# amacati/gp-mpc

Hardware: AMD Instinct MI355X
Metric: GP-MPC control steps/sec, 2D quadrotor H=30 N=200, batch 1024 @1/2/4/8 GPU (higher is better)
Workload: dtype f64

## Files before the change

gp-mpc_amd/csrc/capi.hip:

```cpp
#include "../../include/gpmpc_mi355x.h"

#include <cmath>
#include <cstdio>
#include <cstdlib>
#include <cstring>
#include <string>
#include <unordered_map>
#include <vector>

#include "gp_tile.h"
#include "gpmpc_common.h"

using namespace gpmpc;

static_assert(GPMPC_STATS_SLOTS == kStatsSlots, "public stats-slot count must match the kernel's");

#ifndef GPMPC_VAR_TRIM_DEFAULT
#define GPMPC_VAR_TRIM_DEFAULT 1
#endif

namespace {
thread_local std::string g_err;

gpmpc_status fail(gpmpc_status s, const std::string& msg) {
    g_err = msg;
    return s;
}

#define HIPCHK(expr)                                                                        \
    do {                                                                                    \
        hipError_t e_ = (expr);                                                             \
        if (e_ != hipSuccess)                                                               \
            return fail(GPMPC_ERR_HIP, std::string(#expr) + ": " + hipGetErrorString(e_));   \
    } while (0)

struct ModelDims {
    int nx, nu, ngp, nparams;
    int gp_dim[kMaxGP];
    int var_src[kMaxGP][3];
};

bool model_dims(int id, ModelDims& m) {
    switch (id) {
        case kQuad2D:
            m = ModelDims{6, 2, 2, 6, {1, 3, 0, 0}, {{6, 0, 0}, {4, 5, 7}, {0, 0, 0}, {0, 0, 0}}};
            return true;
        case kQuad3D:
            m = ModelDims{12, 4, 3, 9, {1, 3, 3, 0}, {{0, 0, 0}, {1, 2, 3}, {4, 5, 6}, {0, 0, 0}}};
            return true;
        case kCartpole:
            m = ModelDims{4, 1, 2, 4, {3, 3, 0, 0}, {{2, 3, 4}, {2, 3, 4}, {0, 0, 0}, {0, 0, 0}}};
            return true;
// ... 117 lines not shown
    int32_t* has_prev = nullptr;
    double* lin = nullptr;
    int32_t* lin_tag = nullptr;
    int32_t* t_prev = nullptr;
    bool lin_cache = true;
    int32_t* order = nullptr;
    uint32_t* cost = nullptr;
    double* traj = nullptr;
    double* tgain = nullptr;
    GPSlot gp[kMaxGP];
    bool profiling = false;
    std::vector<hipEvent_t> ev_pool;
    std::unordered_map<hipEvent_t, bool> ev_fenced;
    std::vector<std::pair<hipEvent_t, hipEvent_t>> ev_var, ev_sqp;
    std::vector<hipEvent_t> ev_var_owned;
    unsigned long long* timing = nullptr;
    long long* stats = nullptr;
    int32_t* scratch_i = nullptr;
    double* scratch_d = nullptr;
    double* obs = nullptr;
    double* roll = nullptr;
    size_t roll_doubles = 0;
    double* sel = nullptr;
    size_t sel_rows[kMaxGP] = {0, 0, 0, 0};
    double* red = nullptr;
    size_t red_rows = 0, red_m = 0;
    int var_batch = 0;
    hipStream_t last_stream = nullptr;
    hipEvent_t ev_last = nullptr;
    bool ev_last_valid = false;
    bool tail_unmarked = false;
    bool overlap = true;
    int var_split = 0;
    bool var_trim = GPMPC_VAR_TRIM_DEFAULT != 0;
    bool event_fence = false;
    double* stage_cost = nullptr;
    hipStream_t side = nullptr;
    hipEvent_t ev_fork = nullptr, ev_join = nullptr;
    int tail = -1;
};

static hipError_t order_after_last(gpmpc_handle* h, hipStream_t s) {
    if (!h->ev_last) {
        const hipError_t e = hipEventCreateWithFlags(&h->ev_last, hipEventDisableTiming);
        if (e != hipSuccess) {
            h->ev_last = nullptr;
            return e;
        }
    }
    if (h->last_stream == s) return hipSuccess;
    if (h->tail_unmarked) {
        if (hipEventRecord(h->ev_last, h->last_stream) == hipSuccess) {
            h->ev_last_valid = true;
        } else {
            (void)hipGetLastError();
            (void)hipStreamSynchronize(h->last_stream);
            (void)hipGetLastError();
        }
        h->tail_unmarked = false;
    }
    if (h->ev_last_valid) return hipStreamWaitEvent(s, h->ev_last, 0);
    return hipSuccess;
}
struct StreamMark {
    gpmpc_handle* h;
    hipStream_t s;
    ~StreamMark() {
// ... 1145 lines not shown
    HIPCHK(hipMemcpyAsync(h->u, u_dev, B * H * h->md.nu * sizeof(double), hipMemcpyDeviceToDevice, s));
    bump_lin(h);
    HIPCHK(hipMemsetAsync(h->t_prev, 0xff, B * sizeof(int32_t), s));
    HIPCHK(hipMemsetAsync(h->pi, 0, B * H * h->md.nx * sizeof(double), s));
    HIPCHK(hipMemsetAsync(h->lam, 0, B * (H + 1) * 2 * h->nb * sizeof(double), s));
    return GPMPC_OK;
}

gpmpc_status gpmpc_solve(gpmpc_handle* h, int32_t batch, const double* x0, const int32_t* tstep, double* u0,
                         int32_t* status, int32_t* sqp_iter, int32_t* qp_iter, double* res, void* stream) {
    if (!h) return fail(GPMPC_ERR_ARG, "null handle");
    if (!h->model_set) return fail(GPMPC_ERR_STATE, "gpmpc_set_model not called");
    if (!h->ref_set) return fail(GPMPC_ERR_STATE, "gpmpc_set_reference not called");
    if (batch < 1 || batch > h->max_batch) return fail(GPMPC_ERR_ARG, "batch out of range");
    if (!x0 || !tstep || !u0 || !status) return fail(GPMPC_ERR_ARG, "null output/input");
    if (h->P.tighten && h->P.use_gp)
        for (int g = 0; g < h->md.ngp; ++g)
            if (!h->gp[g].linvT) return fail(GPMPC_ERR_STATE, "tightening needs Linv for every GP");
    (void)hipSetDevice(h->device);
    hipStream_t s = (hipStream_t)stream;
    HIPCHK(order_after_last(h, s));
    StreamMark mark{h, s};
    ProblemDev P = h->P;
    P.tighten = (h->P.tighten && h->P.use_gp) ? 1 : 0;
    auto give_back = [&](hipEvent_t& e) {
        if (e) h->ev_pool.push_back(e);
        e = nullptr;
    };
    auto launch_var = [&](int first, int count, const int32_t* order, hipStream_t st) -> hipError_t {
        PostBatch pb{};
        pb.n = h->md.ngp;
        pb.step_points = batch * h->H;
        pb.var_split = h->var_split;
        pb.var_full = h->var_trim ? 0 : 1;
        for (int g = 0; g < h->md.ngp; ++g) {
            PostArgs& a = pb.a[g];
            a.sx = h->x;
            a.su = h->u;
            a.H = h->H;
            a.nx = h->md.nx;
            a.nu = h->md.nu;
            a.ngp = h->md.ngp;
            a.gp_index = g;
            for (int k = 0; k < 3; ++k) a.src[k] = h->md.var_src[g][k];
            a.P = count * h->H;
            a.d = h->md.gp_dim[g];
            a.with_noise = 1;
            a.mean = nullptr;
            a.var = h->var;
            a.var_stride = h->md.ngp;
            a.var_off = g;
            a.order = order;
            a.first = first;
            pb.g[g] = P.gp[g];
            pb.g[g].vroot = h->gp[g].vroot;
            pb.g[g].vroot_cols = h->gp[g].vroot_cols;
            pb.g[g].vroot_rank = h->gp[g].vroot_rank;
            pb.npad[g] = h->gp[g].npad;
        }
        return launch_gp_post_batch(pb, true, st);
    };
    StateDev S{h->x, h->u, h->pi, h->lam, h->has_prev, h->var, h->tight, h->lin_cache ? h->lin : nullptr, h->lin_tag,
               h->order, h->cost, 0, h->t_prev};
    StepIO io{x0, tstep, u0, status, sqp_iter, qp_iter, res, h->timing, h->stats};
    if (!io.sqp_iter) io.sqp_iter = h->scratch_i;
    if (!io.qp_iter) io.qp_iter = h->scratch_i + h->max_batch;
    if (!io.res) io.res = h->scratch_d;
// ... 155 lines not shown
    }
    return GPMPC_OK;
}

gpmpc_status gpmpc_get_launch_segments(gpmpc_handle* h, int32_t batch, int32_t* segments) {
    if (!h) return fail(GPMPC_ERR_ARG, "null handle");
    if (batch < 1 || batch > h->max_batch) return fail(GPMPC_ERR_ARG, "batch out of range");
    if (!segments) return fail(GPMPC_ERR_ARG, "null output");
    *segments = sqp_launch_segments(h->P, batch);
    return GPMPC_OK;
}

gpmpc_status gpmpc_set_tuning(gpmpc_handle* h, int32_t option, int32_t value) {
    if (!h) return fail(GPMPC_ERR_ARG, "null handle");
    switch (option) {
        case GPMPC_TUNE_LIN_CACHE:
            if (value != 0 && value != 1) break;
            if (h->lin_cache != (value == 1)) bump_lin(h);
            h->lin_cache = value == 1;
            return GPMPC_OK;
        case GPMPC_TUNE_ORDER:
            if (value < 0 || value > 2) break;
            h->P.order_dispatch = value;
            return GPMPC_OK;
        case GPMPC_TUNE_OVERLAP:
            if (value != 0 && value != 1) break;
            h->overlap = value == 1;
            return GPMPC_OK;
        case GPMPC_TUNE_VAR_SPLIT:
            if (value != 0 && value != 1 && value != 4) break;
            h->var_split = value;
            return GPMPC_OK;
        case GPMPC_TUNE_VAR_TRIM:
            if (value != 0 && value != 1) break;
            h->var_trim = value == 1;
            return GPMPC_OK;
        case GPMPC_TUNE_SEG:
            if (value != 0 && value != 1) break;
            h->P.seg = value;
            return GPMPC_OK;
        case GPMPC_TUNE_SEG_PIVOT:
            if (value < -1 || value > 300) break;
            h->P.seg_piv_rel = value < 0 ? HUGE_VAL : std::pow(10.0, -value);
            return GPMPC_OK;
        case GPMPC_TUNE_TAIL:
            if (value < -1 || value > 16384) break;
            h->tail = value;
            return GPMPC_OK;
        case GPMPC_TUNE_SHIFT:
            if (value != 0 && value != 1) break;
            h->P.shift = value;
            return GPMPC_OK;
        case GPMPC_TUNE_EVENT_FENCE:
            if (value != 0 && value != 1) break;
            if (h->event_fence != (value == 1)) {
                for (hipEvent_t e : h->ev_pool) {
                    h->ev_fenced.erase(e);
                    (void)hipEventDestroy(e);
                }
                h->ev_pool.clear();
            }
            h->event_fence = value == 1;
            return GPMPC_OK;
        default:
            return fail(GPMPC_ERR_ARG, "unknown tuning option " + std::to_string(option));
    }
    return fail(GPMPC_ERR_ARG, "bad value " + std::to_string(value) + " for tuning option " + std::to_string(option));
}
// ... 104 lines not shown

gpmpc_status gpmpc_gp_predict(gpmpc_handle* h, int32_t gp_id, const double* Z, int32_t P, double* mean, double* var,
                              int32_t with_noise, void* stream) {
    if (!h) return fail(GPMPC_ERR_ARG, "null handle");
    if (gp_id < 0 || gp_id >= h->md.ngp || !h->gp[gp_id].set) return fail(GPMPC_ERR_STATE, "GP not set");
    if (P < 0 || (P > 0 && !Z)) return fail(GPMPC_ERR_ARG, "bad points");
    if (var && !h->gp[gp_id].linvT) return fail(GPMPC_ERR_STATE, "variance needs Linv");
    if (P == 0) return GPMPC_OK;
    (void)hipSetDevice(h->device);
    hipStream_t s = (hipStream_t)stream;
    HIPCHK(order_after_last(h, s));
    StreamMark mark{h, s};
    const GPDev& g = h->P.gp[gp_id];
    PostArgs a{};
    a.Z = Z;
    a.ldz = h->md.gp_dim[gp_id];
    a.P = P;
    a.d = h->md.gp_dim[gp_id];
    a.with_noise = with_noise;
    a.var_stride = 1;
    a.var_off = 0;
    if (mean) {
        GPDev gm = g;
        gm.vrows = g.rows;
        gm.nv = g.n;
        gm.linvT = nullptr;
        a.mean = mean;
        a.var = nullptr;
        HIPCHK(launch_gp_post(gm, (g.n + 15) / 16 * 16, a, false, s));
    }
    if (var) {
        a.mean = nullptr;
        a.var = var;
        HIPCHK(launch_gp_post(g, h->gp[gp_id].npad, a, false, s, h->var_trim ? 0 : 1));
    }
    return GPMPC_OK;
}

gpmpc_status gpmpc_gp_mean_grad(gpmpc_handle* h, int32_t gp_id, const double* Z, int32_t P, double* mean,
                                double* grad, void* stream) {
    if (!h) return fail(GPMPC_ERR_ARG, "null handle");
    if (gp_id < 0 || gp_id >= h->md.ngp || !h->gp[gp_id].set) return fail(GPMPC_ERR_STATE, "GP not set");
    if (P < 0 || (P > 0 && !Z)) return fail(GPMPC_ERR_ARG, "bad points");
    if (P == 0) return GPMPC_OK;
    (void)hipSetDevice(h->device);
    hipStream_t s = (hipStream_t)stream;
    HIPCHK(order_after_last(h, s));
    StreamMark mark{h, s};
    HIPCHK(launch_gp_mean_grad(h->P.gp[gp_id], Z, P, mean, grad, s));
    return GPMPC_OK;
}

gpmpc_status gpmpc_gp_posterior(int32_t n, int32_t d, int32_t npad, const double* rows, const double* linvT,
                                double lengthscale, double outputscale, double noise, const double* Z, int32_t P,
                                double* mean, double* var, int32_t with_noise, void* stream) {
    if (n < 1 || d < 1 || d > kMaxGPDim || npad < n || npad % 16 != 0 || !rows)
        return fail(GPMPC_ERR_ARG, "bad GP layout (need 1 <= d <= 3, npad = 16-multiple >= n)");
    if (P < 0 || (P > 0 && !Z)) return fail(GPMPC_ERR_ARG, "bad points");
    if (var && !linvT) return fail(GPMPC_ERR_ARG, "variance needs linvT");
    if (!(lengthscale > 0.0) || !(outputscale > 0.0) || !(noise >= 0.0)) return fail(GPMPC_ERR_ARG, "bad hyperparameters");
    if (P == 0) return GPMPC_OK;
    GPDev g{};
    g.rows = rows;
    g.vrows = rows;
    g.linvT = linvT;
    g.n = g.nv = n;
    g.d = d;
// ... 65 lines not shown
    const hipError_t e = hipMalloc(&fresh, doubles * sizeof(double));
    if (e != hipSuccess) return fail(GPMPC_ERR_NOMEM, std::string("hipMalloc: ") + hipGetErrorString(e));
    if (*buf) (void)hipFree(*buf);
    *buf = fresh;
    return GPMPC_OK;
}

static gpmpc_status ensure_observe_scratch(gpmpc_handle* h) {
    return h->obs ? GPMPC_OK : replace_scratch(&h->obs, observe_layout(h).end);
}

struct PointVariances {
    const double* Z;
    int32_t ldz;
    const double* var;
    int32_t ldv;
};
static gpmpc_status queue_point_variances(gpmpc_handle* h, int32_t P, const double* x_dev, const double* u_dev,
                                          hipStream_t s, PointVariances* out) {
    const ObserveLayout lay = observe_layout(h);
    GPObserve a = observe_args(h, P, x_dev, u_dev, nullptr, P, nullptr, 1.0, 0.0);
    a.inputs = h->obs + lay.zin;
    HIPCHK(launch_gp_observe(a, s));
    for (int g = 0, col = 0; g < h->md.ngp; col += h->md.gp_dim[g], ++g) {
        PostArgs pa{};
        pa.Z = h->obs + lay.zin + col;
        pa.ldz = (int)lay.D;
        pa.P = P;
        pa.d = h->md.gp_dim[g];
        pa.with_noise = 0;
        pa.var = h->obs + lay.var + (size_t)g * h->max_batch;
        pa.var_stride = 1;
        pa.var_off = 0;
        HIPCHK(launch_gp_post(h->P.gp[g], h->gp[g].npad, pa, false, s, h->var_trim ? 0 : 1));
    }
    *out = PointVariances{h->obs + lay.zin, (int32_t)lay.D, h->obs + lay.var, h->max_batch};
    return GPMPC_OK;
}

gpmpc_status gpmpc_preprocess(gpmpc_handle* h, int32_t P, const double* x_dev, const double* u_dev,
                              const double* xnext_dev, int32_t m, const int32_t* pick_dev, double dt_diff,
                              double gravity, double* inputs_dev, double* targets_dev, void* stream) {
    if (!h) return fail(GPMPC_ERR_ARG, "null handle");
    const char* bad = transitions_bad(P, x_dev, u_dev, xnext_dev, m, pick_dev, dt_diff, gravity);
    if (!bad && !inputs_dev && !targets_dev) bad = "no output (inputs_dev and targets_dev both NULL)";
    if (bad) return fail(GPMPC_ERR_ARG, bad);
    if (!h->model_set) return fail(GPMPC_ERR_STATE, "the prior parameters are not set (gpmpc_set_model first)");
    (void)hipSetDevice(h->device);
    GPObserve a = observe_args(h, P, x_dev, u_dev, xnext_dev, m, pick_dev, dt_diff, gravity);
    a.inputs = inputs_dev;
    a.targets = targets_dev;
    HIPCHK(launch_gp_observe(a, (hipStream_t)stream));
    return GPMPC_OK;
}

gpmpc_status gpmpc_gp_informative(gpmpc_handle* h, int32_t P, const double* x_dev, const double* u_dev, int32_t m,
                                  int32_t* pick_dev, double* score_dev, void* stream) {
    if (!h) return fail(GPMPC_ERR_ARG, "null handle");
    if (P < 1 || P > h->max_batch) return fail(GPMPC_ERR_ARG, "P must be in 1 .. max_batch");
    if (m < 1 || m > P) return fail(GPMPC_ERR_ARG, "m must be in 1 .. P");
    if (!x_dev || !u_dev || !pick_dev) return fail(GPMPC_ERR_ARG, "null points or picks");
    for (int g = 0; g < h->md.ngp; ++g) {
        if (!h->gp[g].set) return fail(GPMPC_ERR_STATE, "GP not set (gpmpc_set_gp first)");
        if (!h->gp[g].linvT) return fail(GPMPC_ERR_STATE, "the variance needs Linv (the GP was set without it)");
    }
    (void)hipSetDevice(h->device);
    const gpmpc_status got = ensure_observe_scratch(h);
// ... 242 lines not shown
    const size_t need = var_dev ? (size_t)P * T * D : 0;
    if (need > h->roll_doubles) {
        const gpmpc_status got = replace_scratch(&h->roll, need);
        if (got != GPMPC_OK) return got;
        h->roll_doubles = need;
    }
    HIPCHK(ensure_side(h));
    hipStream_t s = h->side;
    HIPCHK(order_after_last(h, s));
    StreamMark mark{h, s};
    RolloutArgs a{};
    for (int i = 0; i < kMaxParams; ++i) a.params[i] = h->P.params[i];
    a.dt = h->P.dt;
    a.P = P;
    a.T = T;
    a.x0 = x0_dev;
    a.u = u_dev;
    a.x = x_dev;
    if (with_gp)
        for (int g = 0; g < ngp; ++g) a.gp[g] = h->P.gp[g];
    HIPCHK(launch_rollout(h->model, a, with_gp != 0, s));
    if (var_dev) {
        HIPCHK(launch_rollout_inputs(h->model, x_dev, u_dev, P, T, h->roll, s));
        for (int g = 0, col = 0; g < ngp; col += h->md.gp_dim[g], ++g) {
            PostArgs pa{};
            pa.Z = h->roll + col;
            pa.ldz = (int)D;
            pa.P = P * T;
            pa.d = h->md.gp_dim[g];
            pa.with_noise = 0;
            pa.var = var_dev;
            pa.var_stride = ngp;
            pa.var_off = g;
            HIPCHK(launch_gp_post(h->P.gp[g], h->gp[g].npad, pa, false, s, h->var_trim ? 0 : 1));
        }
    }
    HIPCHK(hipStreamSynchronize(s));
    return GPMPC_OK;
}

gpmpc_status gpmpc_rollout_lin(gpmpc_handle* h, int32_t P, int32_t T, const double* x0_dev, const double* u_dev,
                               int32_t with_gp, double* x_dev, double* A_dev, double* B_dev, double* var_dev,
                               const double* K, const double* cov0_dev, int32_t with_noise, double* cov_dev) {
    if (!h) return fail(GPMPC_ERR_ARG, "null handle");
    const int nx = h->md.nx, nu = h->md.nu;
    const char* bad = nullptr;
    if (P < 1 || T < 1) bad = "no trajectories or no steps (P, T >= 1)";
    else if (!x0_dev || !u_dev || !x_dev) bad = "null array (x0_dev, u_dev and x_dev are required)";
    else if (!A_dev || !B_dev) bad = "null array (A_dev and B_dev are required)";
    else if (with_gp != 0 && with_gp != 1) bad = "with_gp must be 0 or 1";
    else if (with_noise != 0 && with_noise != 1) bad = "with_noise must be 0 or 1";
    else if ((int64_t)P * ((int64_t)T + 1) * nx > INT32_MAX) bad = "P (T + 1) nx does not fit an int32";
    else if ((int64_t)P * (int64_t)T * nx * nx > INT32_MAX) bad = "P T nx nx does not fit an int32";
    if (!bad && K)
        for (int i = 0; i < nu * nx; ++i)
            if (!std::isfinite(K[i])) bad = "K has a non-finite entry";
    if (bad) return fail(GPMPC_ERR_ARG, bad);
    if (!h->model_set) return fail(GPMPC_ERR_STATE, "the prior parameters are not set (gpmpc_set_model first)");
    const int ngp = h->md.ngp;
    if (with_gp) {
        if (!h->P.use_gp) return fail(GPMPC_ERR_STATE, "with_gp = 1 while the handle's GPs are off (gpmpc_use_gp)");
        for (int g = 0; g < ngp; ++g)
            if (!h->gp[g].set) return fail(GPMPC_ERR_STATE, "GP " + std::to_string(g) + " not set");
    }
    const bool want_var = var_dev || cov_dev;
    if (want_var)
        for (int g = 0; g < ngp; ++g) {
// ... 10 lines not shown
        if (got != GPMPC_OK) return got;
        h->roll_doubles = need;
    }
    HIPCHK(ensure_side(h));
    hipStream_t s = h->side;
    HIPCHK(order_after_last(h, s));
    StreamMark mark{h, s};
    RolloutLinArgs a{};
    for (int i = 0; i < kMaxParams; ++i) a.r.params[i] = h->P.params[i];
    a.r.dt = h->P.dt;
    a.r.P = P;
    a.r.T = T;
    a.r.x0 = x0_dev;
    a.r.u = u_dev;
    a.r.x = x_dev;
    a.A = A_dev;
    a.B = B_dev;
    if (with_gp)
        for (int g = 0; g < ngp; ++g) a.r.gp[g] = h->P.gp[g];
    HIPCHK(launch_rollout_lin(h->model, a, with_gp != 0, s));
    if (want_var) {
        double* var = var_dev ? var_dev : h->roll + gathered;
        HIPCHK(launch_rollout_inputs(h->model, x_dev, u_dev, P, T, h->roll, s));
        for (int g = 0, col = 0; g < ngp; col += h->md.gp_dim[g], ++g) {
            PostArgs pa{};
            pa.Z = h->roll + col;
            pa.ldz = (int)D;
            pa.P = P * T;
            pa.d = h->md.gp_dim[g];
            pa.with_noise = 0;
            pa.var = var;
            pa.var_stride = ngp;
            pa.var_off = g;
            HIPCHK(launch_gp_post(h->P.gp[g], h->gp[g].npad, pa, false, s, h->var_trim ? 0 : 1));
        }
        if (cov_dev) {
            RolloutCovArgs c{};
            c.dt = h->P.dt;
            c.P = P;
            c.T = T;
            c.closed = K ? 1 : 0;
            if (K)
                for (int i = 0; i < nu * nx; ++i) c.K[i] = K[i];
            for (int g = 0; g < ngp; ++g) c.noise[g] = with_noise ? h->P.gp[g].sn2 : 0.0;
            c.x = x_dev;
            c.u = u_dev;
            c.A = A_dev;
            c.B = B_dev;
            c.var = var;
            c.cov0 = cov0_dev;
            c.cov = cov_dev;
            HIPCHK(launch_rollout_cov(h->model, c, s));
        }
    }
    HIPCHK(hipStreamSynchronize(s));
    return GPMPC_OK;
}

gpmpc_status gpmpc_rollout_sample(gpmpc_handle* h, int32_t P, int32_t T, const double* x0_dev, const double* u_dev,
                                  const double* xref_dev, const double* K, int32_t clip, const double* xi_dev,
                                  int32_t with_gp, int32_t with_noise, double* x_dev, double* uapp_dev,
                                  double* var_dev) {
    if (!h) return fail(GPMPC_ERR_ARG, "null handle");
    const int nx = h->md.nx, nu = h->md.nu;
    const char* bad = nullptr;
    if (P < 1 || T < 1) bad = "no trajectories or no steps (P, T >= 1)";
    else if (!x0_dev || !u_dev || !x_dev) bad = "null array (x0_dev, u_dev and x_dev are required)";
// ... 62 lines not shown
```

gp-mpc_amd/csrc/gp_kernels.hip:

```cpp
#include "gpmpc_common.h"
#include "models.h"

#include <algorithm>
#include <atomic>
#include <type_traits>

namespace gpmpc {

typedef double f64x4 __attribute__((ext_vector_type(4)));


template <bool FROM_STATE>
__device__ __forceinline__ void load_point(const PostArgs& a, int p, double (&z)[3]) {
    if (FROM_STATE) {
        const int r = p / a.H, k = p - r * a.H;
        const int b = a.order ? a.order[a.first + r] : r;
#pragma unroll
        for (int dd = 0; dd < 3; ++dd) {
            const int s = a.src[dd];
            z[dd] = (dd < a.d) ? (s < a.nx ? a.sx[((size_t)b * (a.H + 1) + k) * a.nx + s]
                                           : a.su[((size_t)b * a.H + k) * a.nu + (s - a.nx)])
                               : 0.0;
        }
    } else {
#pragma unroll
        for (int dd = 0; dd < 3; ++dd) z[dd] = (dd < a.d) ? a.Z[(size_t)p * a.ldz + dd] : 0.0;
    }
}

constexpr int kPostWaves = 8;
constexpr int kMaxCT = 16;

__device__ __forceinline__ double dpp_quad_sum(double v) {
    auto mv = [](double x, auto ctrl) {
        const long long b = __double_as_longlong(x);
        const int lo = __builtin_amdgcn_update_dpp(0, (int)b, decltype(ctrl)::value, 0xf, 0xf, false);
        const int hi = __builtin_amdgcn_update_dpp(0, (int)(b >> 32), decltype(ctrl)::value, 0xf, 0xf, false);
        return __longlong_as_double(((long long)hi << 32) | (unsigned int)lo);
    };
    v += mv(v, std::integral_constant<int, 0x4E>{});
    v += mv(v, std::integral_constant<int, 0xB1>{});
    return v;
}

__host__ __device__ inline int post_ct(int npad) { return npad / 16 < kMaxCT ? npad / 16 : kMaxCT; }
__host__ __device__ inline int post_stride(int ct) { return 16 * (ct | 1); }

template <bool FROM_STATE, bool FULL>
__global__ __launch_bounds__(64 * kPostWaves) void gp_post_kernel(PostBatch pb) {
    extern __shared__ __attribute__((aligned(16))) double panel[];
    const GPDev& g = pb.g[blockIdx.y];
    const PostArgs& a = pb.a[blockIdx.y];
    const int npad = pb.npad[blockIdx.y];
    if ((int)blockIdx.x * kPostWaves * 16 >= a.P) return;
    const int tid = threadIdx.x;
    const int lane = tid & 63, wave = tid >> 6;
    const int lc = lane & 15;
    const int kq = lane >> 4;
    const int p0 = (blockIdx.x * kPostWaves + wave) * 16;
    const int p = p0 + lc;
    const bool pvalid = p < a.P;
    double z[3];
    load_point<FROM_STATE>(a, pvalid ? p : a.P - 1, z);
    const double c = -0.5 * g.inv_ell2;
    const double4* rows = reinterpret_cast<const double4*>(g.vrows);
    double msum = 0.0;
    auto kval = [&](int i, bool acc_mean) {
        double kv = 0.0;
        if (i < g.nv) {
            const double4 r = rows[i];
            const double xr[3] = {r.x, r.y, r.z};
            double q = 0.0;
#pragma unroll
            for (int dd = 0; dd < 3; ++dd) {
                const double df = (dd < g.d) ? xr[dd] - z[dd] : 0.0;
                q = fma(df, df, q);
// ... 453 lines not shown
    const PostArgs a = pb.a[blockIdx.y];
    const int npad = pb.npad[blockIdx.y];
    const int lane = threadIdx.x & 63, wave = threadIdx.x >> 6;
    const int p0 = (blockIdx.x * kLoveWaves + wave) * 16;
    if (p0 >= a.P) return;
    int nf, nq;
    love_tiles(g.vroot_rank, nf, nq);
    love_dispatch<1, FROM_STATE>(3 * nf + nq, g, a, npad, p0, lane);
}

template <bool FROM_STATE>
hipError_t launch_love(const PostBatch& pb, hipStream_t stream) {
    int blocks = 0;
    for (int q = 0; q < pb.n; ++q) blocks = max(blocks, (pb.a[q].P + 16 * kLoveWaves - 1) / (16 * kLoveWaves));
    hipLaunchKernelGGL((gp_love_kernel<FROM_STATE>), dim3(blocks, pb.n), dim3(64 * kLoveWaves), 0, stream, pb);
    return hipGetLastError();
}

template <int NT, bool FROM_STATE, int NQ>
hipError_t launch_var_tri_nq(const PostBatch& pb, int blocks, hipStream_t stream) {
    static bool attr = false;
    const int lds = 2 * 16 * 16 * (NT | 1) * (int)sizeof(double);
    if (!attr) {
        const hipError_t e = hipFuncSetAttribute((const void*)gp_var_tri_kernel<NT, FROM_STATE, NQ>,
                                                 hipFuncAttributeMaxDynamicSharedMemorySize, lds);
        if (e != hipSuccess) return e;
        attr = true;
    }
    hipLaunchKernelGGL((gp_var_tri_kernel<NT, FROM_STATE, NQ>), dim3(blocks, pb.n), dim3(64 * kPostWaves), lds, stream, pb);
    return hipGetLastError();
}

static int var_tri_quads(const PostBatch& pb, int ntile) {
    if (pb.var_full) return 0;
    int nr = 0;
    for (int q = 0; q < pb.n; ++q) {
        const int r = pb.g[q].nv - 16 * (ntile - 1);
        if (r < 1 || r > 8) return 0;
        nr = std::max(nr, r);
    }
    return (nr + 3) / 4;
}

template <bool FROM_STATE, int NT = 1>
hipError_t launch_var_tri(const PostBatch& pb, int ntile, int blocks, int split, hipStream_t stream) {
    if constexpr (NT <= kMaxCT) {
        if (ntile == NT) {
            if (split == 4) {
                static bool sattr = false;
                const int lds = var_split_lds(NT, split);
                auto* k = gp_var_split_kernel<NT, FROM_STATE, 4>;
                if (!sattr) {
                    const hipError_t e = hipFuncSetAttribute((const void*)k, hipFuncAttributeMaxDynamicSharedMemorySize, lds);
                    if (e != hipSuccess) return e;
                    sattr = true;
                }
                const int pts = 16 * (kPostWaves / split);
                int sblocks = 0;
                for (int q = 0; q < pb.n; ++q) sblocks = std::max(sblocks, (pb.a[q].P + pts - 1) / pts);
                hipLaunchKernelGGL(k, dim3(sblocks, pb.n), dim3(64 * kPostWaves), lds, stream, pb);
                return hipGetLastError();
            }
            switch (var_tri_quads(pb, NT)) {
                case 1: return launch_var_tri_nq<NT, FROM_STATE, 1>(pb, blocks, stream);
                case 2: return launch_var_tri_nq<NT, FROM_STATE, 2>(pb, blocks, stream);
                default: return launch_var_tri_nq<NT, FROM_STATE, 0>(pb, blocks, stream);
            }
        }
        return launch_var_tri<FROM_STATE, NT + 1>(pb, ntile, blocks, split, stream);
    }
    return hipErrorInvalidValue;
}

hipError_t launch_gp_post_batch(const PostBatch& pb, bool from_state, hipStream_t stream) {
    int blocks = 0;
    size_t lds = 0;
    for (int q = 0; q < pb.n; ++q) {
        blocks = max(blocks, (pb.a[q].P + 16 * kPostWaves - 1) / (16 * kPostWaves));
        if (pb.a[q].var != nullptr && (pb.g[q].linvT != nullptr || pb.g[q].vroot != nullptr)) {
            const int ncols = pb.g[q].vroot ? pb.g[q].vroot_cols : pb.npad[q];
            lds = std::max(lds, (size_t)2 * 16 * post_stride(post_ct(ncols)) * sizeof(double));
        }
    }
    if (blocks == 0 || pb.n == 0) return hipSuccess;
    bool love = true;
    for (int q = 0; q < pb.n; ++q) {
        love = love && pb.a[q].mean == nullptr && pb.a[q].var != nullptr && pb.g[q].vroot != nullptr &&
               pb.g[q].vroot_cols % 16 == 0 && pb.g[q].vroot_cols <= 16 * kLoveMaxTiles &&
               pb.g[q].vroot_rank >= 1 && pb.g[q].vroot_rank <= pb.g[q].vroot_cols;
    }
    if (love)
        return from_state ? launch_love<true>(pb, stream) : launch_love<false>(pb, stream);
    bool tri = true;
    for (int q = 0; q < pb.n; ++q)
        tri = tri && pb.a[q].mean == nullptr && pb.a[q].var != nullptr && pb.g[q].linvT != nullptr &&
// ... 5 lines not shown
                n = 256;
            return n;
        }();
        const int step_blocks = pb.step_points > 0 ? (pb.step_points + 16 * kPostWaves - 1) / (16 * kPostWaves) : blocks;
        const int wgs = step_blocks * pb.n;
        int split = 2 * wgs <= ncu ? 4 : 1;
        if (pb.var_split == 1 || pb.var_split == 4) split = pb.var_split;
        return from_state ? launch_var_tri<true>(pb, pb.npad[0] / 16, blocks, split, stream)
                          : launch_var_tri<false>(pb, pb.npad[0] / 16, blocks, split, stream);
    }
    static std::atomic<bool> attr{false};
    if (!attr.load(std::memory_order_acquire)) {
        const int mx = 2 * 16 * post_stride(kMaxCT) * (int)sizeof(double);
        for (const void* k : {(const void*)gp_post_kernel<true, false>, (const void*)gp_post_kernel<false, false>,
                              (const void*)gp_post_kernel<true, true>, (const void*)gp_post_kernel<false, true>}) {
            const hipError_t e = hipFuncSetAttribute(k, hipFuncAttributeMaxDynamicSharedMemorySize, mx);
            if (e != hipSuccess) return e;
        }
        attr.store(true, std::memory_order_release);
    }
    bool full = true;
    for (int q = 0; q < pb.n; ++q) {
        const bool var = pb.a[q].var != nullptr && (pb.g[q].linvT != nullptr || pb.g[q].vroot != nullptr);
        const int ncols = pb.g[q].vroot ? pb.g[q].vroot_cols : pb.npad[q];
        full = full && (!var || post_ct(ncols) == kMaxCT);
    }
    auto* k = from_state ? (full ? gp_post_kernel<true, true> : gp_post_kernel<true, false>)
                         : (full ? gp_post_kernel<false, true> : gp_post_kernel<false, false>);
    hipLaunchKernelGGL(k, dim3(blocks, pb.n), dim3(64 * kPostWaves), lds, stream, pb);
    return hipGetLastError();
}

hipError_t launch_gp_post(const GPDev& g, int npad, const PostArgs& a, bool from_state, hipStream_t stream,
                          int var_full) {
    PostBatch pb{};
    pb.var_full = var_full;
    pb.g[0] = g;
    pb.a[0] = a;
    pb.npad[0] = npad;
    pb.n = 1;
    return launch_gp_post_batch(pb, from_state, stream);
}

template <int ID>
__global__ void plant_step_kernel(PlantParams params, double dt, const double* __restrict__ x,
                                  const double* __restrict__ u, double* __restrict__ xn, int32_t* tstep, int B) {
    using M = Model<ID>;
    constexpr int NX = M::NX, NU = M::NU;
    const int b = blockIdx.x * blockDim.x + threadIdx.x;
    if (b >= B) return;
    double p[kMaxParams];
#pragma unroll
    for (int i = 0; i < kMaxParams; ++i) p[i] = params.v[i];
    double xs[NX], us[NU], k[NX], acc[NX], xi[NX];
    const double gm[kMaxGP] = {0.0, 0.0, 0.0, 0.0};
#pragma unroll
    for (int i = 0; i < NX; ++i) xs[i] = x[(size_t)b * NX + i];
#pragma unroll
    for (int a = 0; a < NU; ++a) us[a] = u[(size_t)b * NU + a];
    const double cs[4] = {0.0, 0.5, 0.5, 1.0}, ws[4] = {1.0, 2.0, 2.0, 1.0};
#pragma unroll
    for (int s = 0; s < 4; ++s) {
#pragma unroll
        for (int i = 0; i < NX; ++i) xi[i] = (s == 0) ? xs[i] : fma(cs[s] * dt, k[i], xs[i]);
        M::f(p, xi, us, gm, k);
#pragma unroll
        for (int i = 0; i < NX; ++i) acc[i] = (s == 0) ? k[i] : fma(ws[s], k[i], acc[i]);
    }
#pragma unroll
// ... 18 lines not shown
```

gp-mpc_amd/csrc/gpmpc_common.h:

```cpp
#pragma once
#include <hip/hip_runtime.h>
#include <cstdint>
#include <type_traits>

namespace gpmpc {

constexpr int kMaxGP = 4;
constexpr int kMaxGPDim = 3;
constexpr int kMaxNX = 12;
constexpr int kMaxNU = 4;
constexpr int kMaxH = 63;
constexpr int kPhases = 15;
constexpr int kMaxParams = 16;
constexpr int kStatsSlots = 12;
constexpr double kSlackMin = 1e-12;

enum ModelId : int32_t { kQuad2D = 0, kQuad3D = 1, kCartpole = 2 };

enum SolveStatus : int32_t { kSuccess = 0, kNaN = 1, kMaxIter = 2, kMinStep = 3, kQPFailure = 4 };

struct GPDev {
    const double* rows;
    const double* vrows;
    const double* linvT;
// ... 116 lines not shown
    p = fma(p, r, 0.5000000000000019);
    p = fma(p, r, 1.0);
    p = fma(p, r, 1.0);
    return __hiloint2double(__double2hiint(p) + (__double2loint(t) << 20), __double2loint(p));
}

template <int K>
__device__ __forceinline__ void exp_rbf_n(double (&x)[K]) {
    constexpr double kMagic = 6755399441055744.0;
    constexpr double c[12] = {2.5110037605963777e-08, 2.763263963904103e-07, 2.755724091857897e-06,
                              2.4801485482328494e-05, 0.00019841269890047113, 0.0013888888952314775,
                              0.008333333333319601, 0.0416666666664881, 0.1666666666666668,
                              0.5000000000000019, 1.0, 1.0};
    double t[K], r[K], p[K];
#pragma unroll
    for (int k = 0; k < K; ++k) x[k] = exp_rbf_clamp(x[k]);
#pragma unroll
    for (int k = 0; k < K; ++k) t[k] = fma(x[k], 1.4426950408889634, kMagic);
#pragma unroll
    for (int k = 0; k < K; ++k) r[k] = fma(t[k] - kMagic, -6.93147180369123816490e-01, x[k]);
#pragma unroll
    for (int k = 0; k < K; ++k) r[k] = fma(t[k] - kMagic, -1.90821492927058770002e-10, r[k]);
#pragma unroll
    for (int k = 0; k < K; ++k) p[k] = fma(c[0], r[k], c[1]);
#pragma unroll
    for (int i = 2; i < 12; ++i)
#pragma unroll
        for (int k = 0; k < K; ++k) p[k] = fma(p[k], r[k], c[i]);
#pragma unroll
    for (int k = 0; k < K; ++k)
        x[k] = __hiloint2double(__double2hiint(p[k]) + (__double2loint(t[k]) << 20), __double2loint(p[k]));
}

__device__ __forceinline__ double dpp_row_sum(double v) {
    auto mv = [](double x, auto ctrl) {
        const long long b = __double_as_longlong(x);
        const int lo = __builtin_amdgcn_update_dpp(0, (int)b, decltype(ctrl)::value, 0xf, 0xf, false);
        const int hi = __builtin_amdgcn_update_dpp(0, (int)(b >> 32), decltype(ctrl)::value, 0xf, 0xf, false);
        return __longlong_as_double(((long long)hi << 32) | (unsigned int)lo);
    };
    v += mv(v, std::integral_constant<int, 0x128>{});
    v += mv(v, std::integral_constant<int, 0x124>{});
    v += mv(v, std::integral_constant<int, 0x4E>{});
    v += mv(v, std::integral_constant<int, 0xB1>{});
    return v;
}

struct PostBatch {
    GPDev g[kMaxGP];
    PostArgs a[kMaxGP];
    int32_t npad[kMaxGP];
    int32_t n;
    int32_t step_points;
    int32_t var_split;
    int32_t var_full;
};

struct GPAppend {
    double* rows;
    double* tX;
    double* tW;
    double* linvT;
    int32_t npad;
    int32_t n0;
    int32_t m;
    int32_t d;
    double xbar[3];
    double inv_ell2, sf2, sn2;
    const double* Xnew;
    const double* ynew;
    double* wt;
    int32_t ldw;
    double* pmean;
    double* lbinv;
    double* beta;
    int32_t* flag;
    int32_t* accepted;
};

struct GPDrop {
    const double* src;
    double* dst;
    const double* rows;
    const double* tX;
    double* srows;
    double* stX;
    double* stW;
    int32_t npad0;
// ... 262 lines not shown
    const double* linvT;
    int32_t nv, npad;
    double inv_ell2, sf2;
};
struct RolloutSampleArgs {
    RolloutArgs r;
    const double* xref;
    const double* xi;
    double* uapp;
    double* var;
    int32_t closed, clip;
    double K[kMaxNU * kMaxNX];
    double u_lo[kMaxNU], u_hi[kMaxNU];
    double noise[kMaxGP];
    RolloutSampleGP vg[kMaxGP];
};
hipError_t launch_rollout_sample(int model, const RolloutSampleArgs& a, bool with_gp, hipStream_t stream);
struct RolloutCovArgs {
    double dt;
    int32_t P, T;
    int32_t closed;
    double K[kMaxNU * kMaxNX];
    double noise[kMaxGP];
    const double* x;
    const double* u;
    const double* A;
    const double* B;
    const double* var;
    const double* cov0;
    double* cov;
};
hipError_t launch_rollout_cov(int model, const RolloutCovArgs& a, hipStream_t stream);
hipError_t launch_gp_post(const GPDev& g, int npad, const PostArgs& a, bool from_state, hipStream_t stream,
                          int var_full = 0);
hipError_t launch_gp_post_batch(const PostBatch& pb, bool from_state, hipStream_t stream);
struct PlantParams {
    double v[kMaxParams];
};
hipError_t launch_plant(int model, const PlantParams& params, double dt, const double* x, const double* u, double* xn,
                        int32_t* tstep, int B, hipStream_t stream);

}
```

gp-mpc_amd/gpmpc/_lib.py:

```python

from __future__ import annotations

import ctypes
import hashlib
import os
from ctypes import POINTER, c_char_p, c_double, c_int32, c_int64, c_void_p
from pathlib import Path

import torch

_DEFAULT_LIB = Path(__file__).resolve().parent / "lib" / "libgpmpc_mi355x.so"
LIB_PATH = Path(os.environ.get("GPMPC_LIB", _DEFAULT_LIB))
CSRC = Path(__file__).resolve().parents[1] / "csrc"
HASHED = ["sqp_kernel.hip", "gp_kernels.hip", "gp_append.hip", "gp_drop.hip", "gp_refactor.hip", "gp_fit.hip",
          "gp_love.hip", "gp_fitc.hip", "gp_observe.hip", "rollout_cov.hip", "capi.hip", "gpmpc_common.h", "gp_tile.h", "gp_pick.h",
          "models.h", "../../include/gpmpc_mi355x.h", "build_id.cpp", "Makefile"]

_lib = None

_D = c_double
_I = c_int32
_P = c_void_p
SIGNATURES = {
    "gpmpc_create": (_I, [_I, _I, _I, _I, POINTER(_P)]),
    "gpmpc_destroy": (None, [_P]),
    "gpmpc_last_error": (c_char_p, []),
    "gpmpc_set_model": (_I, [_P, _P, _I, _D, _P, _P, _P, _P, _P, _P, _P, _D, _I]),
    "gpmpc_set_reference": (_I, [_P, _P, _I]),
    "gpmpc_set_options": (_I, [_P, _I, _D, _D, _D, _D, _I, _D, _D]),
    "gpmpc_set_gp": (_I, [_P, _I, _I, _I, _P, _P, _I, _P, _P, _D, _D, _D]),
    "gpmpc_gp_reserve": (_I, [_P, _I, _I]),
    "gpmpc_gp_append": (_I, [_P, _I, _I, _P, _P, _P, _P]),
    "gpmpc_gp_drop_oldest": (_I, [_P, _I, _I, _P, _P]),
    "gpmpc_gp_drop_rows": (_I, [_P, _I, _I, _P, _P, _P, _P]),
    "gpmpc_gp_refactor": (_I, [_P, _I, _P, _D, _D, _D, _P, _P]),
    "gpmpc_gp_mll": (_I, [_P, _I, _P, _P, _P]),
    "gpmpc_gp_fit": (_I, [_P, _I, _P, _D, _I, POINTER(_D), POINTER(_I), POINTER(_I), _P, _P]),
    "gpmpc_gp_love_root": (_I, [_P, _I, _I, _P, POINTER(_I), POINTER(_I), _P]),
    "gpmpc_get_gp_variance_root": (_I, [_P, _I, POINTER(_I), POINTER(_I), _P, _P]),
    "gpmpc_gp_fitc": (_I, [_P, _I, _I, _P, _P, _D, POINTER(_I), _P]),
    "gpmpc_get_gp_fitc": (_I, [_P, _I, POINTER(_I), _P, _P, _P]),
    "gpmpc_gp_inducing": (_I, [_P, _I, _I, _D, _P, _P, _P, POINTER(_I)]),
    "gpmpc_gp_size": (_I, [_P, _I, POINTER(_I), POINTER(_I)]),
    "gpmpc_use_gp": (_I, [_P, _I]),
    "gpmpc_set_gp_variance_root": (_I, [_P, _I, _I, _I, _P]),
    "gpmpc_set_tightening": (_I, [_P, _I, _D, _P, _P, _P]),
    "gpmpc_set_var_inputs": (_I, [_P, _I, _P, _I]),
    "gpmpc_reset": (_I, [_P, _I, _I, _P]),
# ... 96 lines not shown
```

Before: 3.193 million.

## Add quad-tiled MFMA variance kernel and make it the default trim mode

Adds a new GP posterior-variance kernel that computes the triangular solve product with 4x4x4 f64 MFMA over quad-sized column blocks. It double-buffers Linv panels in LDS and interleaves the RBF kernel-vector evaluation for the next tile with the current tile's MFMAs. A third var_trim mode (2) selects it and becomes the new default. This is meant to cut the wasted work and latency of the older triangular/full variance paths, at the cost of more register pressure, more template instantiations, and a new code path that must match the old numerics.

```diff
diff --git a/gp-mpc_amd/csrc/capi.hip b/gp-mpc_amd/csrc/capi.hip
--- a/gp-mpc_amd/csrc/capi.hip
+++ b/gp-mpc_amd/csrc/capi.hip
@@ -14,10 +14,6 @@
 using namespace gpmpc;
 
 static_assert(GPMPC_STATS_SLOTS == kStatsSlots, "public stats-slot count must match the kernel's");
-
-#ifndef GPMPC_VAR_TRIM_DEFAULT
-#define GPMPC_VAR_TRIM_DEFAULT 1
-#endif
 
 namespace {
 thread_local std::string g_err;
@@ -201,7 +197,7 @@
     bool tail_unmarked = false;
     bool overlap = true;
     int var_split = 0;
-    bool var_trim = GPMPC_VAR_TRIM_DEFAULT != 0;
+    int var_trim = GPMPC_VAR_TRIM_DEFAULT;
     bool event_fence = false;
     double* stage_cost = nullptr;
     hipStream_t side = nullptr;
@@ -1413,7 +1409,7 @@
         pb.n = h->md.ngp;
         pb.step_points = batch * h->H;
         pb.var_split = h->var_split;
-        pb.var_full = h->var_trim ? 0 : 1;
+        pb.var_trim = h->var_trim;
         for (int g = 0; g < h->md.ngp; ++g) {
             PostArgs& a = pb.a[g];
             a.sx = h->x;
@@ -1635,8 +1631,8 @@
             h->var_split = value;
             return GPMPC_OK;
         case GPMPC_TUNE_VAR_TRIM:
-            if (value != 0 && value != 1) break;
-            h->var_trim = value == 1;
+            if (value < 0 || value > 2) break;
+            h->var_trim = value;
             return GPMPC_OK;
         case GPMPC_TUNE_SEG:
             if (value != 0 && value != 1) break;
@@ -1807,7 +1803,7 @@
     if (var) {
         a.mean = nullptr;
         a.var = var;
-        HIPCHK(launch_gp_post(g, h->gp[gp_id].npad, a, false, s, h->var_trim ? 0 : 1));
+        HIPCHK(launch_gp_post(g, h->gp[gp_id].npad, a, false, s, h->var_trim));
     }
     return GPMPC_OK;
 }
@@ -1939,7 +1935,7 @@
         pa.var = h->obs + lay.var + (size_t)g * h->max_batch;
         pa.var_stride = 1;
         pa.var_off = 0;
-        HIPCHK(launch_gp_post(h->P.gp[g], h->gp[g].npad, pa, false, s, h->var_trim ? 0 : 1));
+        HIPCHK(launch_gp_post(h->P.gp[g], h->gp[g].npad, pa, false, s, h->var_trim));
     }
     *out = PointVariances{h->obs + lay.zin, (int32_t)lay.D, h->obs + lay.var, h->max_batch};
     return GPMPC_OK;
@@ -2248,7 +2244,7 @@
             pa.var = var_dev;
             pa.var_stride = ngp;
             pa.var_off = g;
-            HIPCHK(launch_gp_post(h->P.gp[g], h->gp[g].npad, pa, false, s, h->var_trim ? 0 : 1));
+            HIPCHK(launch_gp_post(h->P.gp[g], h->gp[g].npad, pa, false, s, h->var_trim));
         }
     }
     HIPCHK(hipStreamSynchronize(s));
@@ -2325,7 +2321,7 @@
             pa.var = var;
             pa.var_stride = ngp;
             pa.var_off = g;
-            HIPCHK(launch_gp_post(h->P.gp[g], h->gp[g].npad, pa, false, s, h->var_trim ? 0 : 1));
+            HIPCHK(launch_gp_post(h->P.gp[g], h->gp[g].npad, pa, false, s, h->var_trim));
         }
         if (cov_dev) {
             RolloutCovArgs c{};
diff --git a/gp-mpc_amd/csrc/gp_kernels.hip b/gp-mpc_amd/csrc/gp_kernels.hip
--- a/gp-mpc_amd/csrc/gp_kernels.hip
+++ b/gp-mpc_amd/csrc/gp_kernels.hip
@@ -10,38 +10,8 @@
 typedef double f64x4 __attribute__((ext_vector_type(4)));
 
 
-template <bool FROM_STATE>
-__device__ __forceinline__ void load_point(const PostArgs& a, int p, double (&z)[3]) {
-    if (FROM_STATE) {
-        const int r = p / a.H, k = p - r * a.H;
-        const int b = a.order ? a.order[a.first + r] : r;
-#pragma unroll
-        for (int dd = 0; dd < 3; ++dd) {
-            const int s = a.src[dd];
-            z[dd] = (dd < a.d) ? (s < a.nx ? a.sx[((size_t)b * (a.H + 1) + k) * a.nx + s]
-                                           : a.su[((size_t)b * a.H + k) * a.nu + (s - a.nx)])
-                               : 0.0;
-        }
-    } else {
-#pragma unroll
-        for (int dd = 0; dd < 3; ++dd) z[dd] = (dd < a.d) ? a.Z[(size_t)p * a.ldz + dd] : 0.0;
-    }
-}
-
 constexpr int kPostWaves = 8;
 constexpr int kMaxCT = 16;
-
-__device__ __forceinline__ double dpp_quad_sum(double v) {
-    auto mv = [](double x, auto ctrl) {
-        const long long b = __double_as_longlong(x);
-        const int lo = __builtin_amdgcn_update_dpp(0, (int)b, decltype(ctrl)::value, 0xf, 0xf, false);
-        const int hi = __builtin_amdgcn_update_dpp(0, (int)(b >> 32), decltype(ctrl)::value, 0xf, 0xf, false);
-        return __longlong_as_double(((long long)hi << 32) | (unsigned int)lo);
-    };
-    v += mv(v, std::integral_constant<int, 0x4E>{});
-    v += mv(v, std::integral_constant<int, 0xB1>{});
-    return v;
-}
 
 __host__ __device__ inline int post_ct(int npad) { return npad / 16 < kMaxCT ? npad / 16 : kMaxCT; }
 __host__ __device__ inline int post_stride(int ct) { return 16 * (ct | 1); }
@@ -561,7 +531,7 @@
 }
 
 static int var_tri_quads(const PostBatch& pb, int ntile) {
-    if (pb.var_full) return 0;
+    if (pb.var_trim == 0) return 0;
     int nr = 0;
     for (int q = 0; q < pb.n; ++q) {
         const int r = pb.g[q].nv - 16 * (ntile - 1);
@@ -590,6 +560,7 @@
                 hipLaunchKernelGGL(k, dim3(sblocks, pb.n), dim3(64 * kPostWaves), lds, stream, pb);
                 return hipGetLastError();
             }
+            if (pb.var_trim == 2) return launch_var_quad(pb, FROM_STATE, NT, blocks, stream);
             switch (var_tri_quads(pb, NT)) {
                 case 1: return launch_var_tri_nq<NT, FROM_STATE, 1>(pb, blocks, stream);
                 case 2: return launch_var_tri_nq<NT, FROM_STATE, 2>(pb, blocks, stream);
@@ -661,9 +632,9 @@
 }
 
 hipError_t launch_gp_post(const GPDev& g, int npad, const PostArgs& a, bool from_state, hipStream_t stream,
-                          int var_full) {
+                          int var_trim) {
     PostBatch pb{};
-    pb.var_full = var_full;
+    pb.var_trim = var_trim;
     pb.g[0] = g;
     pb.a[0] = a;
     pb.npad[0] = npad;
diff --git a/gp-mpc_amd/csrc/gp_var_quad.h b/gp-mpc_amd/csrc/gp_var_quad.h
--- /dev/null
+++ b/gp-mpc_amd/csrc/gp_var_quad.h
@@ -0,0 +1,210 @@
+#pragma once
+#include "gpmpc_common.h"
+
+#include <algorithm>
+#include <type_traits>
+#include <utility>
+
+namespace gpmpc {
+
+constexpr int kQuadWaves = 4;
+__host__ __device__ constexpr int var_quad_stride(int nt) { return 16 * nt + 4; }
+
+template <class F, int... I>
+__device__ __forceinline__ void static_for_seq(F&& f, std::integer_sequence<int, I...>) {
+    (f(std::integral_constant<int, I>{}), ...);
+}
+template <int N, class F>
+__device__ __forceinline__ void static_for(F&& f) {
+    static_for_seq(f, std::make_integer_sequence<int, N>{});
+}
+
+__host__ __device__ constexpr int quad_first(int q, int ks) { return (4 * q + ks) & ~1; }
+__host__ __device__ constexpr int quad_index(int nq, int q, int ks, int j) {
+    int m = (j - quad_first(q, ks)) / 2;
+    for (int k = 0; k < ks; ++k) m += (nq - quad_first(q, k)) / 2;
+    return m;
+}
+__host__ __device__ constexpr int quad_items(int nq, int q, int nks) { return quad_index(nq, q, nks, quad_first(q, nks)); }
+
+template <int NT, int NQL>
+__global__ __launch_bounds__(64 * kQuadWaves) void gp_var_quad_kernel(PostBatch pb, int from_state) {
+    extern __shared__ __attribute__((aligned(16))) double panel[];
+    constexpr int NQ = 4 * (NT - 1) + NQL;
+    constexpr int NC = 4 * NQ;
+    constexpr int W = var_quad_stride(NT);
+    constexpr int NS = (NC + 31) / 32;
+    const GPDev& g = pb.g[blockIdx.y];
+    const PostArgs& a = pb.a[blockIdx.y];
+    if ((int)blockIdx.x * kQuadWaves * 32 >= a.P) return;
+    const int tid = threadIdx.x;
+    const int lane = tid & 63, wave = tid >> 6;
+    const int lc = lane & 15, kq = lane >> 4;
+    const int p0 = (blockIdx.x * kQuadWaves + wave) * 32;
+    double z[2][3];
+#pragma unroll
+    for (int t = 0; t < 2; ++t) {
+        const int p = p0 + 16 * t + lc;
+        if (from_state) load_point<true>(a, p < a.P ? p : a.P - 1, z[t]);
+        else load_point<false>(a, p < a.P ? p : a.P - 1, z[t]);
+    }
+    const double c = -0.5 * g.inv_ell2, sf2 = g.sf2;
+    constexpr int npad = 16 * NT;
+    const double4* rows = reinterpret_cast<const double4*>(g.vrows);
+    double2 stage[NS];
+    auto fetch = [&](int q) {
+        const int w = NC - 16 * q, nrow = (q == NT - 1) ? 4 * NQL : 16;
+#pragma unroll
+        for (int j = 0; j < NS; ++j) {
+            if (2 * j * 64 * kQuadWaves < nrow * w) {
+                const int e = 2 * (tid + j * 64 * kQuadWaves);
+                const int row = e / w, col = e - row * w;
+                stage[j] = (row < nrow) ? *reinterpret_cast<const double2*>(g.linvT + (size_t)(16 * q + row) * npad + 16 * q + col)
+                                        : double2{0.0, 0.0};
+            }
+        }
+    };
+    auto deposit = [&](int q, double* buf) {
+        const int w = NC - 16 * q, nrow = (q == NT - 1) ? 4 * NQL : 16;
+#pragma unroll
+        for (int j = 0; j < NS; ++j) {
+            if (2 * j * 64 * kQuadWaves < nrow * w) {
+                const int e = 2 * (tid + j * 64 * kQuadWaves);
+                const int row = e / w, col = e - row * w;
+                if (row < nrow) *reinterpret_cast<double2*>(buf + row * W + 16 * q + col) = stage[j];
+            }
+        }
+    };
+    double4 rw[2][4];
+    auto load_rows = [&](int q) {
+#pragma unroll
+        for (int ks = 0; ks < 4; ++ks) rw[q & 1][ks] = rows[16 * q + 4 * ks + kq];
+    };
+    constexpr int kKvSteps = 8 + kExpRbfSteps, kKvOps = 8 * kKvSteps;
+    double ed[8], ex[8], et[8], er[8], ep[8];
+    auto kv_ops = [&](int o0, int n, int par, double (&out)[8]) {
+        const int s = o0 >> 3;
+#pragma unroll
+        for (int u = 0; u < 8; ++u) {
+            if (u < n) {
+                const int k = (o0 & 7) + u, ks = k >> 1, t = k & 1;
+                const double4& x = rw[par][ks];
+                if (s == 0) ed[k] = x.z - z[t][2];
+                else if (s == 1) ex[k] = ed[k] * ed[k];
+                else if (s == 2) ed[k] = x.y - z[t][1];
+                else if (s == 3) ex[k] = fma(ed[k], ed[k], ex[k]);
+                else if (s == 4) ed[k] = x.x - z[t][0];
+                else if (s == 5) ex[k] = fma(ed[k], ed[k], ex[k]);
+                else if (s == 6) ex[k] = c * ex[k];
+                else if (s < 7 + kExpRbfSteps) exp_rbf_step<8>(s - 7, k, ex, et, er, ep);
+                else out[k] = sf2 * ex[k];
+            }
+        }
+    };
+    double acc[2][NQ];
+#pragma unroll
+    for (int j = 0; j < NQ; ++j) acc[0][j] = acc[1][j] = 0.0;
+    fetch(0);
+    load_rows(0);
+    if (NT > 1) load_rows(1);
+    deposit(0, panel);
+    double kv[8];
+#pragma unroll
+    for (int s = 0; s < kKvSteps; ++s) kv_ops(8 * s, 8, 0, kv);
+    __syncthreads();
+    constexpr int kAhead = 4;
+    static_for<NT>([&](auto qc) {
+        constexpr int q = decltype(qc)::value;
+        const double* buf = panel + (q & 1) * 16 * W;
+        constexpr int nks = (q == NT - 1) ? NQL : 4;
+        if constexpr (q + 1 < NT) fetch(q + 1);
+        if constexpr (q + 2 < NT) load_rows(q + 2);
+        constexpr int nitem = quad_items(NQ, q, nks);
+        constexpr int nops = (q + 1 < NT) ? kKvOps : 0, per_item = (2 * q < NT) ? 4 : 8;
+        double kvn[8];
+        double ring[kAhead][2];
+        auto read = [&](int ks, int j, int s) {
+            const double* brow = buf + (4 * ks + kq) * W + (lc & 3);
+            if (j >= 4 * q + ks) ring[s][0] = brow[4 * j];
+            ring[s][1] = brow[4 * j + 4];
+        };
+        static_for<nks>([&](auto kc) {
+            constexpr int ks = decltype(kc)::value;
+            constexpr int f = quad_first(q, ks), cnt = (NQ - f) / 2, base = quad_index(NQ, q, ks, f);
+            constexpr int cprev = ks > 0 ? (NQ - quad_first(q, ks - 1)) / 2 : 0;
+            constexpr int fnext = quad_first(q, ks + 1), cnext = ks + 1 < nks ? (NQ - fnext) / 2 : 0;
+#pragma unroll
+            for (int i = 0; i < kAhead; ++i)
+                if (i < cnt && i + cprev < kAhead) read(ks, f + 2 * i, (base + i) % kAhead);
+#pragma unroll
+            for (int i = 0; i < cnt; ++i) {
+                const int j = f + 2 * i, s = (base + i) % kAhead;
+#pragma unroll
+                for (int h = 0; h < 2; ++h) {
+                    if (j + h >= 4 * q + ks) {
+                        acc[0][j + h] = __builtin_amdgcn_mfma_f64_4x4x4f64(kv[2 * ks], ring[s][h], acc[0][j + h], 0, 0, 0);
+                        acc[1][j + h] = __builtin_amdgcn_mfma_f64_4x4x4f64(kv[2 * ks + 1], ring[s][h], acc[1][j + h], 0, 0, 0);
+                    }
+                }
+                if ((base + i) * per_item < nops) kv_ops((base + i) * per_item, per_item, (q + 1) & 1, kvn);
+                if (i + kAhead < cnt) read(ks, j + 2 * kAhead, s);
+                else if (i + kAhead - cnt < cnext) read(ks + 1, fnext + 2 * (i + kAhead - cnt), s);
+                __builtin_amdgcn_sched_barrier(0);
+            }
+        });
+#pragma unroll
+        for (int s = 0; s < kKvSteps; ++s)
+            if (8 * s >= nitem * per_item && 8 * s < nops) kv_ops(8 * s, 8, (q + 1) & 1, kvn);
+        if constexpr (q + 1 < NT) {
+#pragma unroll
+            for (int i = 0; i < 8; ++i) kv[i] = kvn[i];
+            deposit(q + 1, panel + ((q + 1) & 1) * 16 * W);
+        }
+        __syncthreads();
+    });
+    const double noise = a.with_noise ? g.sn2 : 0.0;
+#pragma unroll
+    for (int t = 0; t < 2; ++t) {
+        double s = 0.0;
+#pragma unroll
+        for (int j = 0; j < NQ; ++j) s = fma(acc[t][j], acc[t][j], s);
+        s = dpp_quad_sum(s);
+        const int pr = p0 + 16 * t + 4 * (lc >> 2) + kq;
+        if ((lc & 3) == 0 && pr < a.P) a.var[post_row(a, pr) * a.var_stride + a.var_off] = sf2 - s + noise;
+    }
+}
+
+template <int NT, int NQL>
+hipError_t launch_var_quad_nql(const PostBatch& pb, bool from_state, int blocks, hipStream_t stream) {
+    static bool attr = false;
+    const int lds = 2 * 16 * var_quad_stride(NT) * (int)sizeof(double);
+    if (!attr) {
+        const hipError_t e = hipFuncSetAttribute((const void*)gp_var_quad_kernel<NT, NQL>,
+                                                 hipFuncAttributeMaxDynamicSharedMemorySize, lds);
+        if (e != hipSuccess) return e;
+        attr = true;
+    }
+    static_assert(kQuadWaves * 32 == 128, "launch_gp_post_batch counts 128-point workgroups");
+    hipLaunchKernelGGL((gp_var_quad_kernel<NT, NQL>), dim3(blocks, pb.n), dim3(64 * kQuadWaves), lds, stream, pb,
+                       from_state ? 1 : 0);
+    return hipGetLastError();
+}
+
+inline int var_quad_last(const PostBatch& pb, int ntile) {
+    int nr = 0;
+    for (int q = 0; q < pb.n; ++q) nr = std::max(nr, pb.g[q].nv - 16 * (ntile - 1));
+    return nr <= 8 ? 2 : 4;
+}
+
+template <int NT>
+hipError_t launch_var_quad_nt(const PostBatch& pb, bool from_state, int ntile, int blocks, hipStream_t stream) {
+    if constexpr (NT <= 16) {
+        if (ntile == NT)
+            return var_quad_last(pb, NT) == 2 ? launch_var_quad_nql<NT, 2>(pb, from_state, blocks, stream)
+                                              : launch_var_quad_nql<NT, 4>(pb, from_state, blocks, stream);
+        return launch_var_quad_nt<NT + 2>(pb, from_state, ntile, blocks, stream);
+    }
+    return hipErrorInvalidValue;
+}
+
+}
diff --git a/gp-mpc_amd/csrc/gp_var_quad.hip b/gp-mpc_amd/csrc/gp_var_quad.hip
--- /dev/null
+++ b/gp-mpc_amd/csrc/gp_var_quad.hip
@@ -0,0 +1,10 @@
+#include "gp_var_quad.h"
+
+namespace gpmpc {
+
+hipError_t launch_var_quad(const PostBatch& pb, bool from_state, int ntile, int blocks, hipStream_t stream) {
+    if (ntile & 1) return launch_var_quad_odd(pb, from_state, ntile, blocks, stream);
+    return launch_var_quad_nt<2>(pb, from_state, ntile, blocks, stream);
+}
+
+}
diff --git a/gp-mpc_amd/csrc/gp_var_quad_odd.hip b/gp-mpc_amd/csrc/gp_var_quad_odd.hip
--- /dev/null
+++ b/gp-mpc_amd/csrc/gp_var_quad_odd.hip
@@ -0,0 +1,9 @@
+#include "gp_var_quad.h"
+
+namespace gpmpc {
+
+hipError_t launch_var_quad_odd(const PostBatch& pb, bool from_state, int ntile, int blocks, hipStream_t stream) {
+    return launch_var_quad_nt<1>(pb, from_state, ntile, blocks, stream);
+}
+
+}
diff --git a/gp-mpc_amd/csrc/gpmpc_common.h b/gp-mpc_amd/csrc/gpmpc_common.h
--- a/gp-mpc_amd/csrc/gpmpc_common.h
+++ b/gp-mpc_amd/csrc/gpmpc_common.h
@@ -172,6 +172,23 @@
         x[k] = __hiloint2double(__double2hiint(p[k]) + (__double2loint(t[k]) << 20), __double2loint(p[k]));
 }
 
+constexpr int kExpRbfSteps = 16;
+template <int K>
+__device__ __forceinline__ void exp_rbf_step(int s, int k, double (&x)[K], double (&t)[K], double (&r)[K], double (&p)[K]) {
+    constexpr double kMagic = 6755399441055744.0;
+    constexpr double c[12] = {2.5110037605963777e-08, 2.763263963904103e-07, 2.755724091857897e-06,
+                              2.4801485482328494e-05, 0.00019841269890047113, 0.0013888888952314775,
+                              0.008333333333319601, 0.0416666666664881, 0.1666666666666668,
+                              0.5000000000000019, 1.0, 1.0};
+    if (s == 0) x[k] = exp_rbf_clamp(x[k]);
+    else if (s == 1) t[k] = fma(x[k], 1.4426950408889634, kMagic);
+    else if (s == 2) r[k] = fma(t[k] - kMagic, -6.93147180369123816490e-01, x[k]);
+    else if (s == 3) r[k] = fma(t[k] - kMagic, -1.90821492927058770002e-10, r[k]);
+    else if (s == 4) p[k] = fma(c[0], r[k], c[1]);
+    else if (s < 15) p[k] = fma(p[k], r[k], c[s - 3]);
+    else x[k] = __hiloint2double(__double2hiint(p[k]) + (__double2loint(t[k]) << 20), __double2loint(p[k]));
+}
+
 __device__ __forceinline__ double dpp_row_sum(double v) {
     auto mv = [](double x, auto ctrl) {
         const long long b = __double_as_longlong(x);
@@ -186,6 +203,40 @@
     return v;
 }
 
+__device__ __forceinline__ double dpp_quad_sum(double v) {
+    auto mv = [](double x, auto ctrl) {
+        const long long b = __double_as_longlong(x);
+        const int lo = __builtin_amdgcn_update_dpp(0, (int)b, decltype(ctrl)::value, 0xf, 0xf, false);
+        const int hi = __builtin_amdgcn_update_dpp(0, (int)(b >> 32), decltype(ctrl)::value, 0xf, 0xf, false);
+        return __longlong_as_double(((long long)hi << 32) | (unsigned int)lo);
+    };
+    v += mv(v, std::integral_constant<int, 0x4E>{});
+    v += mv(v, std::integral_constant<int, 0xB1>{});
+    return v;
+}
+
+template <bool FROM_STATE>
+__device__ __forceinline__ void load_point(const PostArgs& a, int p, double (&z)[3]) {
+    if (FROM_STATE) {
+        const int r = p / a.H, k = p - r * a.H;
+        const int b = a.order ? a.order[a.first + r] : r;
+#pragma unroll
+        for (int dd = 0; dd < 3; ++dd) {
+            const int s = a.src[dd];
+            z[dd] = (dd < a.d) ? (s < a.nx ? a.sx[((size_t)b * (a.H + 1) + k) * a.nx + s]
+                                           : a.su[((size_t)b * a.H + k) * a.nu + (s - a.nx)])
+                               : 0.0;
+        }
+    } else {
+#pragma unroll
+        for (int dd = 0; dd < 3; ++dd) z[dd] = (dd < a.d) ? a.Z[(size_t)p * a.ldz + dd] : 0.0;
+    }
+}
+
+#ifndef GPMPC_VAR_TRIM_DEFAULT
+#define GPMPC_VAR_TRIM_DEFAULT 2
+#endif
+
 struct PostBatch {
     GPDev g[kMaxGP];
     PostArgs a[kMaxGP];
@@ -193,7 +244,7 @@
     int32_t n;
     int32_t step_points;
     int32_t var_split;
-    int32_t var_full;
+    int32_t var_trim;
 };
 
 struct GPAppend {
@@ -522,8 +573,10 @@
 };
 hipError_t launch_rollout_cov(int model, const RolloutCovArgs& a, hipStream_t stream);
 hipError_t launch_gp_post(const GPDev& g, int npad, const PostArgs& a, bool from_state, hipStream_t stream,
-                          int var_full = 0);
+                          int var_trim = GPMPC_VAR_TRIM_DEFAULT);
 hipError_t launch_gp_post_batch(const PostBatch& pb, bool from_state, hipStream_t stream);
+hipError_t launch_var_quad(const PostBatch& pb, bool from_state, int ntile, int blocks, hipStream_t stream);
+hipError_t launch_var_quad_odd(const PostBatch& pb, bool from_state, int ntile, int blocks, hipStream_t stream);
 struct PlantParams {
     double v[kMaxParams];
 };
diff --git a/gp-mpc_amd/gpmpc/_lib.py b/gp-mpc_amd/gpmpc/_lib.py
--- a/gp-mpc_amd/gpmpc/_lib.py
+++ b/gp-mpc_amd/gpmpc/_lib.py
@@ -13,7 +13,8 @@
 LIB_PATH = Path(os.environ.get("GPMPC_LIB", _DEFAULT_LIB))
 CSRC = Path(__file__).resolve().parents[1] / "csrc"
 HASHED = ["sqp_kernel.hip", "gp_kernels.hip", "gp_append.hip", "gp_drop.hip", "gp_refactor.hip", "gp_fit.hip",
-          "gp_love.hip", "gp_fitc.hip", "gp_observe.hip", "rollout_cov.hip", "capi.hip", "gpmpc_common.h", "gp_tile.h", "gp_pick.h",
+          "gp_love.hip", "gp_fitc.hip", "gp_observe.hip", "rollout_cov.hip", "gp_var_quad.hip",
+          "gp_var_quad_odd.hip", "gp_var_quad.h", "capi.hip", "gpmpc_common.h", "gp_tile.h", "gp_pick.h",
           "models.h", "../../include/gpmpc_mi355x.h", "build_id.cpp", "Makefile"]
 
 _lib = None
```

Measured after the change: 3.163 million. No clear change (-1.0%).
